# zepfu/llama-gguf-inference

Hardware: AMD Instinct MI355X
Metric: decode tokens/sec + achieved HBM GB/s, Llama-3-8B Q4_K_M, 1->8 MI355X (higher is better)
Workload: dtype int8; 1 GPU; llama3-8b-q4km: 128-token prompt -> greedy decode on the 128->640 trajectory, 1521 timed tokens at positions 133..1653 (mean context of the trajectory), 1 replica per GPU; model=llama3-8b-q4km, parallelism=replicas x1 (RCCL weight fan-out), global_batch=1

## Files before the change

llama-gguf-inference_amd/csrc/attn.hip:

```cpp
#include "kernels.h"
#include "attn_device.h"
#include "launch_util.h"

#include <cstdlib>

namespace llmi {

template <int D, int G>
__global__ __launch_bounds__(256) void k_attn_scores(AttnArgs a) {
    const int g = blockIdx.x, chunk = blockIdx.y;
    const int n_kv = a.st->pos + 1;
    const int t0 = chunk * 64;
    if (t0 >= n_kv) return;
    const int nt = min(64, n_kv - t0);
    __shared__ float qs[G][D];
    __shared__ __attribute__((aligned(16))) uint16_t ks[64][D + 8];
    for (int i = threadIdx.x; i < G * D; i += 256) qs[i / D][i % D] = h2f(f2h(a.q[(size_t)g * G * D + i]));
    constexpr int PPR = D * 2 / 16;
    const uint16_t* kb = a.kc + ((size_t)g * a.n_ctx + t0) * D;
    for (int i = threadIdx.x; i < nt * PPR; i += 256) {
        const int r = i / PPR, pc = i % PPR;
        *(u32x4*)&ks[r][pc * 8] = *(const u32x4*)(kb + (size_t)r * D + pc * 8);
    }
    __syncthreads();
// ... 585 lines not shown
                const double v = tb + j < n_kv ? (double)f : 0.0;
                if (j & 1) acc1 = __builtin_fma(v, (double)pr[j], acc1);
                else acc0 = __builtin_fma(v, (double)pr[j], acc0);
            }
        }
    }
    double acc = acc0 + acc1;
    acc += xor_partner_d<1>(acc);
    acc += xor_partner_d<2>(acc);
    if constexpr (SLV == 8) acc += xor_partner_d<4>(acc);
    if (sl == 0) a.out[(size_t)h * D + d] = (float)acc;
    LLMI_ATT_STAMP(0, 3)
}

template <int D, int G, int NP>
__global__ __launch_bounds__(256) void k_attl_scores(AttnArgs a) { attl_scores_body<D, G, NP>(a); }
__global__ __launch_bounds__(256) void k_attl_exp(AttnArgs a, int n_head, int kvb) { attl_exp_body(a, n_head, kvb); }
template <int D, int G>
__global__ __launch_bounds__(512) void k_attl_pv(AttnArgs a, int n_head, int kvb) { attl_pv_body<D, G>(a, n_head, kvb); }
template <int D>
__global__ __launch_bounds__(D) void k_attl_sum(AttnArgs a, int n_head) { attl_sum_body<D>(a, n_head); }

template <int D, int P, int S>
__global__ __launch_bounds__(512) void k_attn_d(AttnArgs a, int G, int HK, int kvb, int pf) {
    attn_d_body<D, P, S>(a, G, HK, kvb, pf & 1, (pf >> 1) & 1);
}

int g_xspin_limit = kXSpinLimit;
int g_xtag_skew = 0;

static int g_attn_s = 0;
static int g_attn_pf = 3;
int attn_d_slices(int n_head, int head_dim) {
    const int s = g_attn_s ? g_attn_s : n_head >= 128 ? 2 : n_head >= 64 ? 4 : 8;
    return head_dim / s >= 8 ? s : head_dim / 8;
}

static int g_attn_mode = 0;
void set_attn_mode(int mode) {
    g_attn_mode = mode;
    const char* e = getenv("LLMI_ATTN_S");
    const int v = e ? atoi(e) : 0;
    g_attn_s = (v == 2 || v == 4 || v == 8) ? v : 0;
    const char* f = getenv("LLMI_ATTN_PF");
    g_attn_pf = f ? atoi(f) : 1;
    const char* r = getenv("LLMI_ATTN_ROT");
    if (!r || atoi(r)) g_attn_pf |= 2;
}
// ... 82 lines not shown
    bool ok;
    switch (path) {
        case 1:
            ok = pick([&](auto D) { launch_k(k_attn_fused<D>, heads, dim3(1024), (size_t)kv_bound * 4, s, true, true, a, g, hk); }, d);
            break;
        case 2:
            ok = pick([&](auto D, auto G) {
                launch_k(k_attn_scores8<D, G>, dim3(hk, (kv_bound + 31) / 32), dim3(256), 0, s, true, false, a);
                launch_k(k_attn_pv16<D, G>, dim3(hk, D / 16), dim3(512), lds_g, s, false, true, a, kv_bound);
            }, d, gq);
            break;
        case 4:
            ok = pick([&](auto D, auto G, auto NP) {
                if constexpr (D == 64 || NP < 4)
                    launch_k(k_attn_x<D, G, NP>, dim3(hk, D / 16), dim3(512), lds_g, s, true, true, a, kv_bound);
            }, d, gq, Of<1, 2, 4>{attn_x_np(head_dim, kv_bound)});
            break;
        case 5:
            ok = pick([&](auto D, auto P) { launch_k(k_attn_r<D, P>, heads, dim3(512), 0, s, true, true, a, g, kv_bound); },
                      d, Of<1, 2, 4, 8>{attn_passes(kv_bound, 8)});
            break;
        case 6:
            ok = pick([&](auto D, auto P, auto S) {
                launch_k(k_attn_d<D, P, S>, dim3(n_head * S), dim3(512), 0, s, true, true, a, g, hk, kv_bound, g_attn_pf);
            }, d, Of<1, 2, 4, 8, 12, 16>{attn_passes(kv_bound, 16)}, Of<2, 4, 8>{attn_d_slices(n_head, head_dim)});
            break;
        case 7:
            ok = pick([&](auto D, auto G, auto NP) {
                launch_k(k_attl_scores<D, G, NP>, dim3(hk, lg.nscores), dim3(256), 0, s, true, false, a);
                launch_k(k_attl_exp, dim3(n_head, lg.ntile), dim3(256), 0, s, false, false, a, n_head, kv_bound);
                launch_k(k_attl_pv<D, G>, dim3(hk, lg.ntile), dim3(512), 0, s, false, false, a, n_head, kv_bound);
                launch_k(k_attl_sum<D>, heads, dim3(D), 0, s, false, true, a, n_head);
            }, d, gq, Of<1, 4>{lg.np});
            break;
        default:
            ok = pick([&](auto D, auto G) {
                launch_k(k_attn_scores<D, G>, dim3(hk, (kv_bound + 63) / 64), dim3(256), 0, s, true, false, a);
                launch_k(k_attn_pv<D, G>, dim3(hk, D / 16), dim3(256), 0, s, false, true, a);
            }, d, gq);
    }
    return ok ? hipGetLastError() : hipErrorInvalidValue;
}

}
```

llama-gguf-inference_amd/csrc/attn_device.h:

```cpp
#pragma once

#include "mv_device.h"

namespace llmi {

#if defined(LLMI_EXP_TRACE)
#define LLMI_ATT_STAMP(K, I)                                                                      \
    if (a.trace && (threadIdx.x & 63) == 0)                                                       \
        a.trace[((size_t)(K) * 4096 + blockIdx.y * gridDim.x + blockIdx.x) * 64 + (threadIdx.x >> 6) * 4 + (I)] = \
            __builtin_amdgcn_s_memrealtime();
#else
#define LLMI_ATT_STAMP(K, I)
#endif

template <int D, int G>
__device__ __forceinline__ void attn_scores8_body(const AttnArgs& a) {
    LLMI_ATT_STAMP(0, 0)
    const int g = blockIdx.x, tile = blockIdx.y, t0 = tile * 32;
    const int tid = threadIdx.x, lane = tid & 63, wave = tid >> 6;
    constexpr int DQ = D / 8;
    const int t = t0 + (tid >> 3), qd = tid & 7;
    const uint16_t* kr = a.kc + ((size_t)g * a.n_ctx + t) * D + qd * DQ;
    u32x4 kv[DQ / 8];
#pragma unroll
// ... 344 lines not shown
        if constexpr (SL == 8) v += xor_partner_d<4>(v);
        if (sl == 0) part[((size_t)(g * G + hh) * ntl + tile) * D + d] = v;
    }
}

template <int D>
__device__ __forceinline__ void attl_sum_body(const AttnArgs& a, int n_head) {
    const int h = blockIdx.x, d = threadIdx.x;
    const int n_kv = a.st->pos + 1;
    const int ntl = (a.n_ctx + kLongTile - 1) / kLongTile, ntv = (n_kv + kLongTile - 1) / kLongTile;
    const double* part = attl_part(a, n_head) + (size_t)h * ntl * D + d;
    double s = 0.0;
    for (int j0 = 0; j0 < ntv; j0 += 16) {
        double v[16];
#pragma unroll
        for (int k = 0; k < 16; ++k) v[k] = part[(size_t)min(j0 + k, ntl - 1) * D];
#pragma unroll
        for (int k = 0; k < 16; ++k)
            if (j0 + k < ntv) s += v[k];
    }
    a.out[(size_t)h * D + d] = (float)s;
}

template <int D, int P, int S>
__device__ __forceinline__ void attn_d_body(const AttnArgs& a, int G, int HK, int kvb, int pf = 0, int rot_on = 0) {
    constexpr int DQ = D / 8;
    constexpr int DS = D / S;
    constexpr int SLV = 512 / DS;
    constexpr int NVL = (64 * P + 8 * SLV - 1) / (8 * SLV);
    static_assert(SLV <= 64 && (SLV & (SLV - 1)) == 0, "PV lanes of a dim stay in one wave");
    __shared__ __attribute__((aligned(16))) float sp[64 * P + 8];
    __shared__ float redm[8];
    __shared__ double reds[8];
    LLMI_ATT_STAMP(0, 0)
    const int b = blockIdx.x, H = HK * G;
    const int g = b % HK, h = g * G + (b / HK) % G, ds = b / H;
    const int tid = threadIdx.x, lane = tid & 63, wave = tid >> 6;
    const int qd = tid & 7, pp = tid >> 3;
    const int pos = a.st->pos;
    const int lim = pf ? pos + 1 : kvb;
    const int rot = rot_on ? (b / HK) % P : 0;
    auto pb = [&](int p) { return p + rot < P ? p + rot : p + rot - P; };
    float4 qv[DQ / 4];
#pragma unroll
    for (int i = 0; i < DQ / 4; ++i) qv[i] = *(const float4*)(a.q + (size_t)h * D + qd * DQ + 4 * i);
    u32x4 kv[P][DQ / 8];
#pragma unroll
    for (int p = 0; p < P; ++p) {
        const int t = min(64 * pb(p) + pp, kvb - 1);
        const uint16_t* kr = a.kc + ((size_t)g * a.n_ctx + t) * D + qd * DQ;
        if (64 * pb(p) < lim) {
#pragma unroll
            for (int i = 0; i < DQ / 8; ++i) kv[p][i] = *(const u32x4*)(kr + 8 * i);
        } else {
#pragma unroll
            for (int i = 0; i < DQ / 8; ++i) kv[p][i] = u32x4{0u, 0u, 0u, 0u};
        }
    }
    const int d = ds * DS + tid / SLV, sl = tid % SLV;
    const uint16_t* vr = a.vc + ((size_t)g * D + d) * a.n_ctx;
    u32x4 vv[NVL];
#pragma unroll
    for (int u = 0; u < NVL; ++u) {
        if (8 * SLV * u < lim) vv[u] = *(const u32x4*)(vr + min(8 * sl + 8 * SLV * u, kvb - 8));
        else vv[u] = u32x4{0u, 0u, 0u, 0u};
    }
    const int n_kv = pos + 1;
    double q[DQ];
#pragma unroll
    for (int i = 0; i < DQ / 4; ++i) {
        q[4 * i + 0] = (double)h2f(f2h(qv[i].x)); q[4 * i + 1] = (double)h2f(f2h(qv[i].y));
        q[4 * i + 2] = (double)h2f(f2h(qv[i].z)); q[4 * i + 3] = (double)h2f(f2h(qv[i].w));
    }
    float m = -INFINITY;
#pragma unroll
    for (int p = 0; p < P; ++p) {
        if (64 * pb(p) >= lim) continue;
        double acc = 0.0;
#pragma unroll
        for (int i = 0; i < DQ / 8; ++i)
#pragma unroll
            for (int jj = 0; jj < 4; ++jj) {
                acc = __builtin_fma((double)h2f((uint16_t)kv[p][i][jj]), q[8 * i + 2 * jj], acc);
                acc = __builtin_fma((double)h2f((uint16_t)(kv[p][i][jj] >> 16)), q[8 * i + 2 * jj + 1], acc);
            }
        acc += xor_partner_d<1>(acc);
        acc += xor_partner_d<2>(acc);
        acc += xor_partner_d<4>(acc);
        const int t = 64 * pb(p) + pp;
// ... 66 lines not shown
```

llama-gguf-inference_amd/csrc/battn.hip:

```cpp
#include "kernels.h"
#include "attn_device.h"
#include "launch_util.h"

namespace llmi {

template <int D, int G>
__global__ __launch_bounds__(256) void k_battn_scores8(BAttnArgs b) {
    const AttnArgs a = b.a[blockIdx.z];
    attn_scores8_body<D, G>(a);
}
template <int D, int G>
__global__ __launch_bounds__(512) void k_battn_pv16(BAttnArgs b, int kvb) {
    const AttnArgs a = b.a[blockIdx.z];
    attn_pv16_body<D, G>(a, kvb);
}
template <int D, int P, int S>
__global__ __launch_bounds__(512) void k_battn_d(BAttnArgs b, int G, int HK, int kvb) {
    attn_d_body<D, P, S>(b.a[blockIdx.y], G, HK, kvb, 1, 1);
}
template <int D, int G, int NP>
__global__ __launch_bounds__(256) void k_battl_scores(BAttnArgs b) { attl_scores_body<D, G, NP>(b.a[blockIdx.z]); }
__global__ __launch_bounds__(256) void k_battl_exp(BAttnArgs b, int n_head, int kvb) { attl_exp_body(b.a[blockIdx.z], n_head, kvb); }
template <int D, int G>
__global__ __launch_bounds__(512) void k_battl_pv(BAttnArgs b, int n_head, int kvb) { attl_pv_body<D, G>(b.a[blockIdx.z], n_head, kvb); }
template <int D>
__global__ __launch_bounds__(D) void k_battl_sum(BAttnArgs b, int n_head) { attl_sum_body<D>(b.a[blockIdx.z], n_head); }

hipError_t launch_battention(const BAttnArgs& b, int nt, int n_head, int n_head_kv, int head_dim, int kv_bound,
                             hipStream_t s) {
    if (nt < 1 || nt > kMaxBatch || n_head_kv <= 0 || n_head % n_head_kv) return hipErrorInvalidValue;
    if (b.a[0].fa) return launch_battention_fa(b, nt, n_head, n_head_kv, head_dim, kv_bound, s);
    if (b.a[0].num) return launch_battention_x86(b, nt, n_head, n_head_kv, head_dim, kv_bound, s);
    const int g = n_head / n_head_kv, hk = n_head_kv;
    const OfD d{head_dim};
    const OfG gq{g};
    const LongGeo lg = attn_long_geo(kv_bound);
    bool ok = false;
    switch (battn_path(g, n_head, head_dim, kv_bound, nt)) {
        case 2:
            ok = pick([&](auto D, auto G) {
                hipLaunchKernelGGL((k_battn_scores8<D, G>), dim3(hk, (kv_bound + 31) / 32, nt), dim3(256), 0, s, b);
// ... 23 lines not shown
```

llama-gguf-inference_amd/csrc/mv_device.h:

```cpp
#pragma once

#include <hip/hip_runtime.h>

#include "kernels.h"
#include "../../include/llmi_math.h"

namespace llmi {

typedef unsigned int u32x4 __attribute__((ext_vector_type(4)));
typedef unsigned int u32x2 __attribute__((ext_vector_type(2)));
typedef int i32x4 __attribute__((ext_vector_type(4)));
typedef short short2_t __attribute__((ext_vector_type(2)));

#ifndef LLMI_NT
#define LLMI_NT 1
#endif
constexpr bool kNontemporalWeights = LLMI_NT != 0;

__device__ __forceinline__ float h2f(uint32_t h) {
    return (float)__builtin_bit_cast(_Float16, (uint16_t)(h & 0xffffu));
}
__device__ __forceinline__ uint16_t f2h(float f) {
    __asm__("" : "+v"(f));
    return __builtin_bit_cast(uint16_t, (_Float16)f);
// ... 178 lines not shown
        for (int j = 0; j < 16; ++j) am = fmaxf(am, fabsf(v[j]));
        am = fmaxf(am, xor_partner<1>(am));
        const float d = am / 127;
        if constexpr (X86) {
            const float id = am != 0.f ? 127.f / am : 0.0f;
#pragma unroll
            for (int j = 0; j < 16; ++j) q[j] = (int)__builtin_rintf(v[j] * id);
        } else {
            const float id = d != 0.f ? 1.0f / d : 0.0f;
#pragma unroll
            for (int j = 0; j < 16; ++j) q[j] = (int)roundf(v[j] * id);
        }
        uint8_t* rec = L.act + (size_t)(sb >> 4) * kRec;
        if ((sb & 1) == 0) *(float*)(rec + kRecBs + 2 * (sb & 15)) = h2f(f2h(d));
        u32x4 pk;
#pragma unroll
        for (int w = 0; w < 4; ++w)
            pk[w] = (uint32_t)(q[4 * w] & 0xff) | ((uint32_t)(q[4 * w + 1] & 0xff) << 8) |
                    ((uint32_t)(q[4 * w + 2] & 0xff) << 16) | ((uint32_t)(q[4 * w + 3] & 0xff) << 24);
        *(u32x4*)(rec + 16 * (sb & 15)) = pk;
    }
}

template <bool NORM, int NP>
struct ProRegs {
    float x[NP][16];
    float w[NORM ? NP : 1][16];
};
template <bool NORM, int NP, int NT = kMVThreads>
__device__ __forceinline__ void mv_prologue_issue(const MVArgs& A, ProRegs<NORM, NP>& R) {
    const int nsub = A.cols / 16;
#pragma unroll
    for (int i = 0; i < NP; ++i) {
        const int sb = min((int)threadIdx.x + i * NT, nsub - 1);
#pragma unroll
        for (int k = 0; k < 4; ++k) {
            const float4 xv = *(const float4*)(A.x + sb * 16 + 4 * k);
            R.x[i][4 * k + 0] = xv.x; R.x[i][4 * k + 1] = xv.y; R.x[i][4 * k + 2] = xv.z; R.x[i][4 * k + 3] = xv.w;
            if constexpr (NORM) {
                const float4 wv = *(const float4*)(A.nw + sb * 16 + 4 * k);
                R.w[i][4 * k + 0] = wv.x; R.w[i][4 * k + 1] = wv.y; R.w[i][4 * k + 2] = wv.z; R.w[i][4 * k + 3] = wv.w;
            }
        }
    }
}
template <bool NORM, int NP>
__device__ __forceinline__ void load_sub(const MVArgs& A, const ProRegs<NORM, NP>& R, int i, int sb, float (&v)[16],
                                         float (&w)[16]) {
    if (i < NP) {
#pragma unroll
        for (int ii = 0; ii < NP; ++ii)
            if (ii == i) {
#pragma unroll
// ... 51 lines not shown
            float v[16];
#pragma unroll
            for (int j = 0; j < 16; ++j) {
                v[j] = R.x[i][j];
                if constexpr (NORM) v[j] = (v[j] * scale) * R.w[i][j];
            }
            quant_sub<ACT, X86>(L, cols, sb, v);
        }
    }
    for (int sb = tid + NP * NT; sb < nsub; sb += NT) {
        float v[16], w[16];
        load_sub<NORM, NP>(A, R, NP, sb, v, w);
        if constexpr (NORM) {
#pragma unroll
            for (int j = 0; j < 16; ++j) v[j] = (v[j] * scale) * w[j];
        }
        quant_sub<ACT, X86>(L, cols, sb, v);
    }
}
template <int NI>
struct ImgRegs {
    u32x4 v[NI];
};
template <int NI, int NT = kMVThreads>
__device__ __forceinline__ void mv_img_issue(const MVArgs& A, ImgRegs<NI>& R) {
    const int n16 = (A.cols >> 8) * (kRec / 16);
#pragma unroll
    for (int i = 0; i < NI; ++i) R.v[i] = *(const u32x4*)(A.xq + 16 * min((int)threadIdx.x + i * NT, n16 - 1));
}
template <int NI, int NT = kMVThreads>
__device__ __forceinline__ void mv_img_finish(const MVArgs& A, const Lds& L, const ImgRegs<NI>& R) {
    const int n16 = (A.cols >> 8) * (kRec / 16);
#pragma unroll
    for (int i = 0; i < NI; ++i)
        if ((int)threadIdx.x + i * NT < n16) ((u32x4*)L.act)[threadIdx.x + i * NT] = R.v[i];
    for (int i = (int)threadIdx.x + NI * NT; i < n16; i += NT) ((u32x4*)L.act)[i] = *(const u32x4*)(A.xq + 16 * i);
}

template <int ACT, bool NORM, int X86 = 0>
__device__ __forceinline__ void mv_prologue(const MVArgs& A, const Lds& L) {
    ProRegs<NORM, 1> R;
    mv_prologue_issue<NORM, 1>(A, R);
    mv_prologue_finish<ACT, NORM, 1, kMVThreads, X86>(A, L, R);
}

constexpr uint32_t M4 = 0x0F0F0F0Fu, M2 = 0x03030303u, M1 = 0x01010101u;

__device__ __forceinline__ void scale_min(int j, uint32_t s0, uint32_t s1, uint32_t s2, int& sc, int& m) {
// ... 460 lines not shown

__device__ __forceinline__ float x86_v_expf(float x) {
    const float r = 0x1.8p23f;
    const float z = __builtin_fmaf(x, 0x1.715476p+0f, r);
    const float n = z - r;
    const float b = __builtin_fmaf(-n, 0x1.7f7d1cp-20f, __builtin_fmaf(-n, 0x1.62e4p-1f, x));
    const uint32_t e = __float_as_uint(z) << 23;
    const float k = __uint_as_float(e + __float_as_uint(1.0f));
    const float u = b * b;
    const float j = __builtin_fmaf(__builtin_fmaf(__builtin_fmaf(0x1.0e4020p-7f, b, 0x1.573e2ep-5f), u,
                                                  __builtin_fmaf(0x1.555e66p-3f, b, 0x1.fffdb6p-2f)),
                                   u, 0x1.ffffecp-1f * b);
    if (!(fabsf(n) > 126.f)) return __builtin_fmaf(j, k, k);
    const uint32_t g = n <= 0.f ? 0x82000000u : 0u;
    const float s1 = __uint_as_float(g + 0x7f000000u), s2 = __uint_as_float(e - g);
    if (fabsf(n) > 192.f) return s1 * s1;
    return __builtin_fmaf(s2, j, s2) * s1;
}
__device__ __forceinline__ float x86_silu(float x) { return x / (1.0f + x86_v_expf(-x)); }

struct TaskGeo {
    int lr, R, nj, U;
};
__host__ __device__ inline TaskGeo task_geo(const MVArgs& A) {
    TaskGeo g;
    g.lr = A.lr;
    g.R = A.rpt;
    g.U = A.cols >> 8;
    g.nj = (g.U + g.lr - 1) / g.lr;
    return g;
}

__host__ __device__ constexpr int q80_rs(int lr) { return 8 * lr + 4; }

template <int ACT>
__device__ __forceinline__ void fold_sub(float* F, int R, int lr, int n, bool last, float& acc) {
    constexpr int NC = row_chains<ACT>();
    const int lane = threadIdx.x & 63, nf = R * NC;
    const int len = ACT ? 8 * n : n, stride = ACT ? q80_rs(lr) : kq_cs(lr);
    for (int f = lane; f < nf; f += 64) {
        float a = chain_batched(len, acc, ChainAdd{F + f * stride});
        if (last) {
            F[kFoldF + f] = a;
            a = 0.f;
        }
        acc = a;
    }
// ... 245 lines not shown
        if constexpr (X86) {
            if constexpr (ACT == 1) {
                unit_store_x86<T_Q8_0>(load_unit<T_Q8_0>(sg, lu.row, lu.u, g.U), rec, F, r, ul, g.lr, g.R, lu.valid);
            } else {
                switch (sg.type) {
                    case T_Q4_K: unit_store_x86<T_Q4_K>(load_unit<T_Q4_K>(sg, lu.row, lu.u, g.U), rec, F, r, ul, g.lr, g.R, lu.valid); break;
                    case T_Q5_K: unit_store_x86<T_Q5_K>(load_unit<T_Q5_K>(sg, lu.row, lu.u, g.U), rec, F, r, ul, g.lr, g.R, lu.valid); break;
                    default: unit_store_x86<T_Q6_K>(load_unit<T_Q6_K>(sg, lu.row, lu.u, g.U), rec, F, r, ul, g.lr, g.R, lu.valid); break;
                }
            }
        } else if constexpr (ACT == 1) {
            unit_terms<T_Q8_0>(load_unit<T_Q8_0>(sg, lu.row, lu.u, g.U), rec, tm);
        } else {
            switch (sg.type) {
                case T_Q4_K: unit_terms<T_Q4_K>(load_unit<T_Q4_K>(sg, lu.row, lu.u, g.U), rec, tm); break;
                case T_Q5_K: unit_terms<T_Q5_K>(load_unit<T_Q5_K>(sg, lu.row, lu.u, g.U), rec, tm); break;
                default: unit_terms<T_Q6_K>(load_unit<T_Q6_K>(sg, lu.row, lu.u, g.U), rec, tm); break;
            }
        }
        sub_finish<ACT, EPI, MA, X86>(A, F, g, s, b, sg, tm, lu, r, ul, acc, vg, pos, best);
    }
}

__host__ __device__ inline TaskGeo task_geo_split(const MVArgs& A, int lanes, int R) {
    TaskGeo g;
    g.lr = lanes >> 1;
    g.R = R;
    g.U = A.cols >> 8;
    g.nj = (g.U + g.lr - 1) / g.lr;
    return g;
}
template <int T>
struct HalfW {
    u32x4 q[4];
    u32x4 s;
    u32x4 h[2];
    uint32_t d;
};
template <int T>
__device__ __forceinline__ HalfW<T> load_half(const Seg& sg, uint32_t row, uint32_t u, uint32_t U, uint32_t half) {
    static_assert(T == T_Q4_K || T == T_Q6_K, "split units: Q4_K and Q6_K");
    HalfW<T> w;
    const uint32_t P = (U * 16) << sg.rgs, ru = row * U + u;
    const uint32_t oa = piece_off(row, 0, u, U, 8, sg.rgs) + 4 * half * P;
#pragma unroll
    for (int p = 0; p < 4; ++p) w.q[p] = ldw(sg.a + oa + (uint32_t)p * P);
    if constexpr (T == T_Q4_K) {
// ... 216 lines not shown
```

llama-gguf-inference_amd/csrc/mv_kernels.h:

```cpp
#pragma once
#include "kernels.h"
#include "launch_util.h"
#include "mv_device.h"

#include <algorithm>
#include <cstdlib>
#include <map>
#include <mutex>
#include <tuple>
#include <type_traits>

namespace llmi {

#ifndef LLMI_MV_PINGPONG
#define LLMI_MV_PINGPONG 1
#endif
#ifndef LLMI_Q6_MASKED
#define LLMI_Q6_MASKED 1
#endif
constexpr bool kQ6Masked = LLMI_Q6_MASKED != 0;
__host__ inline size_t mv_lds_total(int act, int cols, int nw, int t, int t2, int x86 = 0) {
    const int ff = fold_stride_cols(act, x86, cols);
    const size_t base = fold_off(act, cols, nw) + (size_t)nw * ff * 4;
    return base + ((kQ6Masked && !x86 && (t == T_Q6_K || t2 == T_Q6_K)) ? (size_t)(cols >> 8) * kQ6MaskRec : 0);
}

static int g_split_by_pairs = getenv("LLMI_SPLIT_BY_PAIRS") ? atoi(getenv("LLMI_SPLIT_BY_PAIRS")) : 0;


#if defined(LLMI_EXP_TRACE)
#define MV_STAMP(I, V)                                                                                    \
    if (A.trace && (threadIdx.x & 63) == 0)                                                               \
        A.trace[((size_t)blockIdx.x * (NT / 64) + (threadIdx.x >> 6)) * 16 + (I)] = (V);
#define MV_NOW __builtin_amdgcn_s_memrealtime()
#else
#define MV_STAMP(I, V)
#endif

template <int ACT, bool NORM, int EPI, int T, int NP, int NT = kMVThreads, int X86 = 0, int US = 1>
__device__ __forceinline__ unsigned long long mv_body(const MVArgs& A, const Lds& L, float* F, const TaskGeo& g, int t0,
                                                      int G, int tbeg, int tend) {
    using W = std::conditional_t<US == 2, HalfW<US == 2 ? T : T_Q4_K>, UnitW<T>>;
    int pos = 0;
    if constexpr (EPI == EPI_QKV) pos = A.st->pos;
    unsigned long long best = 0;
    const int lane = threadIdx.x & 63;
    const int S = EPI == EPI_SWIGLU ? 2 * g.nj : g.nj;
    const int slot = US == 2 ? lane >> 1 : lane;
    [[maybe_unused]] const uint32_t half = lane & 1;
    const int r = slot / g.lr, ul = slot - r * g.lr;
    const auto load = [&](const Seg& s, uint32_t row, uint32_t u) {
        if constexpr (US == 2) return load_half<T>(s, row, u, g.U, half);
        else return load_unit<T>(s, row, u, g.U);
    };

    int task = t0;
    MV_STAMP(0, MV_NOW)
    [[maybe_unused]] int nsub_done = 0, nsub_alt = 0;
    ProRegs<NORM, NP> R;
    ImgRegs<2 * NP + 1> RI;
    const bool img = A.xq != nullptr;
    if (img) mv_img_issue<2 * NP + 1, NT>(A, RI);
    else mv_prologue_issue<NORM, NP, NT>(A, R);
    if ((tend - tbeg <= G && A.xfirst >= 0) || A.xfirst > 0) asm volatile("s_waitcnt vmcnt(0)" ::: "memory");
    const bool pipe = task < tend && task_is<EPI, T>(A, g, task);
    Sub b = sub_of<EPI>(A, g, task < tend ? task : tend - 1, 0);
    Seg sg = pick(A, b.si);
    LaneUnit lu = lane_unit(g, b, sg, r, ul);
    W cur = load(sg, pipe ? lu.row : 0u, pipe ? lu.u : 0u);
    if (img) mv_img_finish<2 * NP + 1, NT>(A, L, RI);
    else mv_prologue_finish<ACT, NORM, NP, NT, X86>(A, L, R);
    __syncthreads();
    [[maybe_unused]] uint8_t* q6m = nullptr;
    if constexpr (T == T_Q6_K && kQ6Masked && !X86) {
        q6m = (uint8_t*)L.act + fold_off(ACT, A.cols, NT / 64) + (size_t)(NT / 64) * kFoldFloats * 4;
        q6_masks_build<NT>(L, g.U, q6m);
        __syncthreads();
    }
    MV_STAMP(1, MV_NOW)

    if (pipe) {
        int s = 0;
        float acc = 0.f, vg = 0.f;
        bool first_sub = A.fw != 0;
        auto step = [&](W& cur, W& nxt) -> bool {
            int tn = task, sn = s + 1;
            Sub bn = b;
            Seg sgn = sg;
            bool has_next = true;
            if (sn == S) {
                sn = 0;
                tn = task + G;
                has_next = tn < tend && task_is<EPI, T>(A, g, tn);
            }
            if (has_next) {
                bn = sub_of<EPI>(A, g, tn, sn);
                sgn = pick(A, bn.si);
            }
// ... 39 lines not shown
            return true;
        };
#if LLMI_MV_PINGPONG
        W other;
        for (;;) {
            if (!step(cur, other)) break;
            if (!step(other, cur)) break;
        }
#else
        for (;;) {
            W nxt;
            if (!step(cur, nxt)) break;
            cur = nxt;
        }
#endif
    }
    if constexpr (US == 1)
        for (; task < tend; task += G) task_any<ACT, EPI, MVArgs, X86>(A, L, F, g, task, r, ul, pos, best);
    MV_STAMP(3, MV_NOW)
    MV_STAMP(5, ((unsigned long long)(__builtin_amdgcn_s_getreg(6164) & 15) << 32) | (unsigned)nsub_done)
    return best;
}

template <int ACT, bool NORM, int EPI, int T, int NP, int T2 = T, int NT = kMVThreads, int X86 = 0>
__global__ __launch_bounds__(NT) void k_matvec(MVArgs A) {
    constexpr int NW = NT / 64;
    extern __shared__ __attribute__((aligned(16))) uint8_t smem[];
    const Lds L = carve(smem, ACT, A.cols);
    const int wave = uniform((int)(threadIdx.x >> 6));
    const int lane = threadIdx.x & 63;
    float* F = (float*)(smem + fold_off(ACT, A.cols, NW)) + wave * fold_stride(ACT, X86, A.rpt, A.lr);
    unsigned long long best;
    if constexpr (T2 == T) {
        int t0 = blockIdx.x * NW + wave, G = gridDim.x * NW, tb = 0, te = A.ntasks;
        if (A.split_wgs > 0) {
            if ((int)blockIdx.x < A.split_wgs) {
                G = A.split_wgs * NW;
                te = A.split_tasks;
            } else {
                t0 = A.split_tasks + (blockIdx.x - A.split_wgs) * NW + wave;
                G = (gridDim.x - A.split_wgs) * NW;
                tb = A.split_tasks;
            }
        }
        best = mv_body<ACT, NORM, EPI, T, NP, NT, X86>(A, L, F, task_geo(A), t0, G, tb, te);
    } else {
        if ((int)blockIdx.x < A.split_wgs)
            best = mv_body<ACT, NORM, EPI, T, NP, NT, X86>(A, L, F, task_geo(A), blockIdx.x * NW + wave, A.split_wgs * NW, 0, A.split_tasks);
        else
            best = mv_body<ACT, NORM, EPI, T2, NP, NT, X86>(A, L, F, task_geo(A), A.split_tasks + (blockIdx.x - A.split_wgs) * NW + wave,
                                                            (gridDim.x - A.split_wgs) * NW, A.split_tasks, A.ntasks);
    }
    if constexpr (EPI == EPI_LOGITS) {
        const int cur_pos = A.st->pos;
        unsigned long long* red = (unsigned long long*)L.red;
        best = wave_max_u64(best);
        __syncthreads();
        if (lane == 0) red[wave] = best;
        __syncthreads();
        if (threadIdx.x == 0) {
            unsigned long long b = red[0];
#pragma unroll
            for (int w = 1; w < NW; ++w) b = red[w] > b ? red[w] : b;
            if (b) atomicMax(&A.argmax[(cur_pos & 1) * kArgSlots + blockIdx.x % kArgSlots], b);
            if (blockIdx.x == 0) A.st->pos_next = cur_pos + 1;
        }
    }
}

template <typename K>
static dim3 resident_grid(K kernel, dim3 grid, size_t lds, int threads = kMVThreads) {
    static std::mutex mu;
    static std::map<std::tuple<const void*, size_t, int>, int> cache;
    int dev = 0;
    (void)hipGetDevice(&dev);
    const auto key = std::make_tuple((const void*)kernel, lds, dev * 4096 + threads);
    int cap = 0;
    {
        std::lock_guard<std::mutex> lk(mu);
        auto it = cache.find(key);
        if (it != cache.end()) {
            cap = it->second;
        } else {
            int occ = 0, cus = 0;
            if (hipOccupancyMaxActiveBlocksPerMultiprocessor(&occ, kernel, threads, lds) != hipSuccess || occ <= 0) occ = 1;
            if (hipDeviceGetAttribute(&cus, hipDeviceAttributeMultiprocessorCount, dev) != hipSuccess || cus <= 0) cus = 1;
            cap = occ * cus;
            cache.emplace(key, cap);
        }
    }
// ... 9 lines not shown
    return v;
}
static inline int wide_cols() {
    static const int v = [] {
        const char* e = getenv("LLMI_MV_WIDE");
        return e ? atoi(e) : 12288;
    }();
    return v;
}
static inline int wide_epis() {
    static const int v = [] {
        const char* e = getenv("LLMI_MV_WIDE_EPI");
        return e ? atoi(e) : (1 << EPI_ADD) | (1 << EPI_SWIGLU) | (1 << EPI_QKV);
    }();
    return v;
}
constexpr int kMVWide = 512;
template <int ACT, bool NORM, int T, int EPI, int NP, int X86>
static hipError_t mv_launch_wide(const MVArgs& a, hipStream_t s) {
    constexpr int NW = kMVWide / 64;
    const size_t lds = mv_lds_total(ACT, a.cols, NW, T, T, X86);
    if (lds > 160 * 1024) return hipErrorInvalidValue;
    const int blocks = std::max(1, std::min(cu_count(), (a.ntasks + NW - 1) / NW));
    launch_k(k_matvec<ACT, NORM, EPI, T, NP, T, kMVWide, X86>, dim3(blocks), dim3(kMVWide), lds, s, true, true, a);
    return hipGetLastError();
}
template <int ACT, bool NORM, int T, int EPI, int X86>
static bool mv_try_wide(const MVArgs& a, hipStream_t s, hipError_t& e) {
    if constexpr ((EPI == EPI_ADD || EPI == EPI_SWIGLU || EPI == EPI_QKV || EPI == EPI_LOGITS) && !(X86 && ACT)) {
        const int wc = wide_cols();
        if (wc <= 0 || a.cols < wc || cu_count() <= 0 || !(wide_epis() >> EPI & 1)) return false;
        for (int i = 0; i < a.nseg; ++i)
            if (a.seg[i].type != T) return false;
        const int per = (a.cols / 16 + kMVWide - 1) / kMVWide;
        e = per <= 1 ? mv_launch_wide<ACT, NORM, T, EPI, 1, X86>(a, s)
            : per <= 2 ? mv_launch_wide<ACT, NORM, T, EPI, 2, X86>(a, s) : mv_launch_wide<ACT, NORM, T, EPI, 4, X86>(a, s);
        return true;
    } else {
        (void)a; (void)s; (void)e;
        return false;
    }
}
constexpr int kMVNarrow = 64;
static inline int narrow_on() {
    static const int v = getenv("LLMI_MV_NARROW") ? atoi(getenv("LLMI_MV_NARROW")) : 1;
    return v;
}
static inline int narrow_tpc() {
    static const int v = getenv("LLMI_MV_NARROW_TPC") ? atoi(getenv("LLMI_MV_NARROW_TPC")) : kMVWaves;
    return v;
}
template <int ACT, bool NORM, int T, int EPI, int NP, int X86>
static hipError_t mv_launch_narrow(const MVArgs& a0, hipStream_t s) {
    const size_t lds = mv_lds_total(ACT, a0.cols, 1, T, T, X86);
    if (lds > 160 * 1024) return hipErrorInvalidValue;
    auto k = k_matvec<ACT, NORM, EPI, T, NP, T, kMVNarrow, X86>;
    const dim3 g = resident_grid(k, dim3(a0.ntasks), lds, kMVNarrow);
    MVArgs a = a0;
    a.split_wgs = 0;
    launch_k(k, g, dim3(kMVNarrow), lds, s, true, true, a);
    return hipGetLastError();
}
template <int ACT, bool NORM, int T, int EPI, int X86>
static bool mv_try_narrow(const MVArgs& a, hipStream_t s, hipError_t& e) {
    if constexpr (EPI == EPI_ADD || EPI == EPI_SWIGLU || EPI == EPI_QKV || EPI == EPI_STORE) {
        const int cus = cu_count();
        if (!narrow_on() || cus <= 0 || a.ntasks >= cus * narrow_tpc()) return false;
        for (int i = 0; i < a.nseg; ++i)
            if (a.seg[i].type != T) return false;
        const int per = (a.cols / 16 + kMVNarrow - 1) / kMVNarrow;
        e = per <= 2 ? mv_launch_narrow<ACT, NORM, T, EPI, 2, X86>(a, s) : mv_launch_narrow<ACT, NORM, T, EPI, 4, X86>(a, s);
        return true;
    } else {
        (void)a; (void)s; (void)e;
        return false;
    }
}
template <int ACT, bool NORM, int T, int EPI, int NP, int X86>
static hipError_t mv_launch(const MVArgs& a0, dim3 grid, size_t lds_in, hipStream_t s) {
    const size_t lds = std::max(lds_in, mv_lds_total(ACT, a0.cols, kMVWaves, T, T, X86));
    if (lds > 160 * 1024) return hipErrorInvalidValue;
    auto k = k_matvec<ACT, NORM, EPI, T, NP, T, kMVThreads, X86>;
    const dim3 g = resident_grid(k, grid, lds);
    MVArgs a = a0;
    a.split_wgs = 0;
    const double sh = old_share();
    const int cus = cu_count();
    if (sh > 0 && cus > 0 && (int)g.x == 2 * cus && a.ntasks >= 4 * (int)g.x * kMVWaves) {
        a.split_wgs = cus;
        a.split_tasks = (int)(a.ntasks * (sh / (1.0 + sh)) + 0.5);
    }
    launch_k(k, g, dim3(kMVThreads), lds, s, true, true, a);
    return hipGetLastError();
}

static inline int split_groups(int wgs, int p1, int p2, double b1, double b2) {
    int best = 1;
    double best_cost = 1e300;
    for (int w1 = 1; w1 < wgs; ++w1) {
        const int n1 = w1 * kMVWaves, n2 = (wgs - w1) * kMVWaves;
        const double c = std::max((double)((p1 + n1 - 1) / n1) * b1, (double)((p2 + n2 - 1) / n2) * b2);
        if (c < best_cost) { best_cost = c; best = w1; }
    }
    return best;
}
template <int ACT, bool NORM, int T, int T2, int EPI, int NP, int X86>
static hipError_t mv_launch2(const MVArgs& a0, int split_tasks, dim3 grid, size_t lds_in, hipStream_t s) {
    const size_t lds = std::max(lds_in, mv_lds_total(ACT, a0.cols, kMVWaves, T, T2, X86));
    if (lds > 160 * 1024) return hipErrorInvalidValue;
    auto k = k_matvec<ACT, NORM, EPI, T, NP, T2, kMVThreads, X86>;
    const dim3 g = resident_grid(k, grid, lds);
    MVArgs a = a0;
    a.split_tasks = split_tasks;
    int w1;
    if (g_split_by_pairs) {
        w1 = (int)(((long long)g.x * split_tasks + a.ntasks / 2) / a.ntasks);
        w1 = w1 < 1 ? 1 : w1 > (int)g.x - 1 ? (int)g.x - 1 : w1;
    } else {
        w1 = split_groups((int)g.x, split_tasks, a.ntasks - split_tasks, (double)tensor_bytes(T, a.rpt, a.cols),
                          (double)tensor_bytes(T2, a.rpt, a.cols));
    }
    a.split_wgs = w1;
    launch_k(k, g, dim3(kMVThreads), lds, s, true, true, a);
    return hipGetLastError();
}

static inline int prologue_np(int cols) {
    const int per = (cols / 16 + kMVThreads - 1) / kMVThreads;
    return per <= 1 ? 1 : per <= 2 ? 2 : 4;
}

template <int ACT, bool NORM, int T, int EPI, int X86>
static hipError_t mv_launch_np(const MVArgs& a, dim3 grid, size_t lds, hipStream_t s) {
    hipError_t e = hipSuccess;
    if (mv_try_wide<ACT, NORM, T, EPI, X86>(a, s, e)) return e;
    if (mv_try_narrow<ACT, NORM, T, EPI, X86>(a, s, e)) return e;
    switch (prologue_np(a.cols)) {
        case 1: return mv_launch<ACT, NORM, T, EPI, 1, X86>(a, grid, lds, s);
        case 2: return mv_launch<ACT, NORM, T, EPI, 2, X86>(a, grid, lds, s);
        default: return mv_launch<ACT, NORM, T, EPI, 4, X86>(a, grid, lds, s);
    }
}

template <int ACT, bool NORM, int T, int X86>
hipError_t mv_dispatch_epi(const MVArgs& a, int epi, dim3 grid, size_t lds, hipStream_t s) {
    switch (epi) {
        case EPI_STORE: return mv_launch_np<ACT, NORM, T, EPI_STORE, X86>(a, grid, lds, s);
        case EPI_ADD: return mv_launch_np<ACT, NORM, T, EPI_ADD, X86>(a, grid, lds, s);
        default: break;
    }
    if constexpr (NORM) {
        switch (epi) {
            case EPI_QKV: return mv_launch_np<ACT, NORM, T, EPI_QKV, X86>(a, grid, lds, s);
            case EPI_SWIGLU: return mv_launch_np<ACT, NORM, T, EPI_SWIGLU, X86>(a, grid, lds, s);
            case EPI_LOGITS: return mv_launch_np<ACT, NORM, T, EPI_LOGITS, X86>(a, grid, lds, s);
            default: break;
        }
    }
    return hipErrorInvalidValue;
}

template <bool NORM, int T, int T2, int X86>
hipError_t mv_qkv2_launch(const MVArgs& a, int split_tasks, dim3 grid, size_t lds, hipStream_t s) {
    return mv_launch2<0, NORM, T, T2, EPI_QKV, 1, X86>(a, split_tasks, grid, lds, s);
}

template <bool NORM, int EPI, int T, int T2, int NT, int X86, int US, int US2>
__global__ __launch_bounds__(NT) void k_matvec_split(MVArgs A) {
    constexpr int NW = NT / 64;
    extern __shared__ __attribute__((aligned(16))) uint8_t smem[];
    const Lds L = carve(smem, 0, A.cols);
    const int wave = uniform((int)(threadIdx.x >> 6));
    float* F = (float*)(smem + fold_off(0, A.cols, NW)) + wave * fold_stride(0, X86, 1, 4);
    if constexpr (T2 == T) {
        static_assert(US == 2 && US2 == 2, "single-type split launches split every unit");
        mv_body<0, NORM, EPI, T, 1, NT, X86, 2>(A, L, F, task_geo_split(A, A.lr, A.rpt), blockIdx.x * NW + wave,
                                                 gridDim.x * NW, 0, A.ntasks);
    } else {
        if ((int)blockIdx.x < A.split_wgs) {
            const TaskGeo g = US == 2 ? task_geo_split(A, A.lr, A.rpt) : task_geo(A);
            mv_body<0, NORM, EPI, T, 1, NT, X86, US>(A, L, F, g, blockIdx.x * NW + wave, A.split_wgs * NW, 0, A.split_tasks);
        } else {
            const int bi = (int)blockIdx.x - A.split_wgs, nb2 = (int)gridDim.x - A.split_wgs;
            TaskGeo g = task_geo_split(A, A.lr2, A.rpt2);
            if constexpr (US2 == 1) {
                g.lr = A.lr2;
                g.nj = (g.U + g.lr - 1) / g.lr;
            }
            mv_body<0, NORM, EPI, T2, 1, NT, X86, US2>(A, L, F, g, A.t2beg + bi * NW + wave, nb2 * NW, A.t2beg, A.t2end);
        }
    }
}

template <bool NORM, int EPI, int T, int NT, int X86>
static hipError_t mv_split_launch_nt(const MVArgs& a, hipStream_t s) {
    constexpr int NW = NT / 64;
    const size_t lds = mv_lds_total(0, a.cols, NW, T, T, X86);
    if (lds > 160 * 1024) return hipErrorInvalidValue;
    auto k = k_matvec_split<NORM, EPI, T, T, NT, X86, 2, 2>;
    const dim3 g = resident_grid(k, dim3((a.ntasks + NW - 1) / NW), lds, NT);
    launch_k(k, g, dim3(NT), lds, s, true, true, a);
    return hipGetLastError();
}
template <bool NORM, int T, int X86>
hipError_t mv_split_launch(const MVArgs& a, int epi, int nt, hipStream_t s) {
    if (a.us != 2 || (nt != 256 && nt != 512)) return hipErrorInvalidValue;
    for (int i = 0; i < a.nseg; ++i)
        if (a.seg[i].type != T) return hipErrorInvalidValue;
#define LLMI_SPLIT_NT(E_) (nt == 512 ? mv_split_launch_nt<NORM, E_, T, 512, X86>(a, s) : mv_split_launch_nt<NORM, E_, T, 256, X86>(a, s))
    if (epi == EPI_STORE) return LLMI_SPLIT_NT(EPI_STORE);
    if (epi == EPI_ADD) return LLMI_SPLIT_NT(EPI_ADD);
    if constexpr (NORM)
        if (epi == EPI_QKV) return LLMI_SPLIT_NT(EPI_QKV);
#undef LLMI_SPLIT_NT
    return hipErrorInvalidValue;
}

static inline int split_groups_nw(int wgs, int nw, int p1, int p2, double b1, double b2) {
    int best = 1;
    double best_cost = 1e300;
    for (int w1 = 1; w1 < wgs; ++w1) {
        const int n1 = w1 * nw, n2 = (wgs - w1) * nw;
        const double c = std::max((double)((p1 + n1 - 1) / n1) * b1, (double)((p2 + n2 - 1) / n2) * b2);
        if (c < best_cost) { best_cost = c; best = w1; }
    }
    return best;
}
template <int NT, int X86, int US>
static hipError_t mv_split_qkv2_launch_nt(const MVArgs& a0, hipStream_t s) {
    constexpr int NW = NT / 64;
    const size_t lds = mv_lds_total(0, a0.cols, NW, T_Q4_K, T_Q6_K, X86);
    if (lds > 160 * 1024) return hipErrorInvalidValue;
    auto k = k_matvec_split<true, EPI_QKV, T_Q4_K, T_Q6_K, NT, X86, US, 2>;
    MVArgs a = a0;
    const int p1 = a.split_tasks, p2 = a.t2end - a.t2beg;
    const dim3 g = resident_grid(k, dim3((p1 + NW - 1) / NW + (p2 + NW - 1) / NW), lds, NT);
    if (g.x < 2) return hipErrorInvalidValue;
    a.split_wgs = split_groups_nw((int)g.x, NW, p1, p2, US == 2 ? 1.0 : 2.0, 2.4);
    launch_k(k, g, dim3(NT), lds, s, true, true, a);
    return hipGetLastError();
}
template <int X86, int US>
hipError_t mv_split_qkv2_launch(const MVArgs& a, int nt, hipStream_t s) {
    if (a.us != US || a.us2 != 2 || a.nseg < 2 || a.cols > 16 * 256 || (nt != 256 && nt != 512)) return hipErrorInvalidValue;
    return nt == 512 ? mv_split_qkv2_launch_nt<512, X86, US>(a, s) : mv_split_qkv2_launch_nt<256, X86, US>(a, s);
}

}
```

Measured before the change: 536.0 tokens/s.

## Hoist kernel-argument loads and overlap step-position read with early K-cache loads

Kernel arguments for the attention and matvec kernels are flattened into leading scalar parameters, so the hot fields sit at the front of the kernarg segment and can be loaded as scalars without pulling in the whole struct. In attention, the step position is now requested through an explicit scalar load, and for deep pass counts the K rows already known to be live are loaded before waiting on that position. The aim is to hide the latency of the dependent pos load and of the argument fetch at kernel start. The cost is more complex code with inline asm, a sched_barrier, and a 'live = kvb-256' margin that assumes pos never trails kvb by more than 256.

```diff
diff --git a/llama-gguf-inference_amd/csrc/attn.hip b/llama-gguf-inference_amd/csrc/attn.hip
--- a/llama-gguf-inference_amd/csrc/attn.hip
+++ b/llama-gguf-inference_amd/csrc/attn.hip
@@ -631,8 +631,12 @@
 __global__ __launch_bounds__(D) void k_attl_sum(AttnArgs a, int n_head) { attl_sum_body<D>(a, n_head); }
 
 template <int D, int P, int S>
-__global__ __launch_bounds__(512) void k_attn_d(AttnArgs a, int G, int HK, int kvb, int pf) {
-    attn_d_body<D, P, S>(a, G, HK, kvb, pf & 1, (pf >> 1) & 1);
+__global__ __launch_bounds__(512) void k_attn_d(const float* q, const uint16_t* kc, const uint16_t* vc, const StepState* st,
+                                                float* out, int n_ctx, int geo, int kvb, float scale,
+                                                unsigned long long* trace) {
+    const int pf = geo >> 24;
+    attn_d_body<D, P, S>(AttnDArgs{q, kc, vc, st, out, n_ctx, scale, trace}, geo & 255, (geo >> 8) & 0xffff, kvb, pf & 1,
+                         (pf >> 1) & 1);
 }
 
 int g_xspin_limit = kXSpinLimit;
@@ -761,7 +765,8 @@
             break;
         case 6:
             ok = pick([&](auto D, auto P, auto S) {
-                launch_k(k_attn_d<D, P, S>, dim3(n_head * S), dim3(512), 0, s, true, true, a, g, hk, kv_bound, g_attn_pf);
+                launch_k(k_attn_d<D, P, S>, dim3(n_head * S), dim3(512), 0, s, true, true, a.q, a.kc, a.vc, a.st, a.out,
+                         a.n_ctx, g | hk << 8 | g_attn_pf << 24, kv_bound, a.scale, a.trace);
             }, d, Of<1, 2, 4, 8, 12, 16>{attn_passes(kv_bound, 16)}, Of<2, 4, 8>{attn_d_slices(n_head, head_dim)});
             break;
         case 7:
diff --git a/llama-gguf-inference_amd/csrc/attn_device.h b/llama-gguf-inference_amd/csrc/attn_device.h
--- a/llama-gguf-inference_amd/csrc/attn_device.h
+++ b/llama-gguf-inference_amd/csrc/attn_device.h
@@ -390,8 +390,32 @@
     a.out[(size_t)h * D + d] = (float)s;
 }
 
+struct AttnDArgs {
+    const float* q;
+    const uint16_t* kc;
+    const uint16_t* vc;
+    const StepState* st;
+    float* out;
+    int n_ctx;
+    float scale;
+    unsigned long long* trace;
+};
+__device__ __forceinline__ AttnDArgs attn_d_args(const AttnArgs& a) {
+    return {a.q, a.kc, a.vc, a.st, a.out, a.n_ctx, a.scale, a.trace};
+}
+
+__device__ __forceinline__ int step_pos_request(const StepState* st) {
+    int pos;
+    asm volatile("s_load_dword %0, %1, %2" : "=s"(pos) : "s"(st), "n"(offsetof(StepState, pos)));
+    return pos;
+}
+__device__ __forceinline__ int step_pos_wait(int pos) {
+    asm volatile("s_waitcnt lgkmcnt(0)" : "+s"(pos));
+    return pos;
+}
+
 template <int D, int P, int S>
-__device__ __forceinline__ void attn_d_body(const AttnArgs& a, int G, int HK, int kvb, int pf = 0, int rot_on = 0) {
+__device__ __forceinline__ void attn_d_body(const AttnDArgs& a, int G, int HK, int kvb, int pf = 0, int rot_on = 0) {
     constexpr int DQ = D / 8;
     constexpr int DS = D / S;
     constexpr int SLV = 512 / DS;
@@ -400,29 +424,45 @@
     __shared__ __attribute__((aligned(16))) float sp[64 * P + 8];
     __shared__ float redm[8];
     __shared__ double reds[8];
+    const int pos_req = step_pos_request(a.st);
     LLMI_ATT_STAMP(0, 0)
     const int b = blockIdx.x, H = HK * G;
     const int g = b % HK, h = g * G + (b / HK) % G, ds = b / H;
     const int tid = threadIdx.x, lane = tid & 63, wave = tid >> 6;
     const int qd = tid & 7, pp = tid >> 3;
-    const int pos = a.st->pos;
-    const int lim = pf ? pos + 1 : kvb;
+    const int live = kvb - 256;
     const int rot = rot_on ? (b / HK) % P : 0;
     auto pb = [&](int p) { return p + rot < P ? p + rot : p + rot - P; };
     float4 qv[DQ / 4];
 #pragma unroll
     for (int i = 0; i < DQ / 4; ++i) qv[i] = *(const float4*)(a.q + (size_t)h * D + qd * DQ + 4 * i);
     u32x4 kv[P][DQ / 8];
+    auto k_row = [&](int p) {
+        const int t = min(64 * pb(p) + pp, kvb - 1);
+        return a.kc + ((size_t)g * a.n_ctx + t) * D + qd * DQ;
+    };
+    constexpr bool EARLY = P > 4;
+    if constexpr (EARLY) {
+#pragma unroll
+        for (int p = 0; p < P; ++p) {
+            if (64 * pb(p) + 64 <= live) {
+                const uint16_t* kr = k_row(p);
+#pragma unroll
+                for (int i = 0; i < DQ / 8; ++i) kv[p][i] = *(const u32x4*)(kr + 8 * i);
+            } else {
+#pragma unroll
+                for (int i = 0; i < DQ / 8; ++i) kv[p][i] = u32x4{0u, 0u, 0u, 0u};
+            }
+        }
+    }
+    const int pos = step_pos_wait(pos_req);
+    const int lim = pf ? pos + 1 : kvb;
 #pragma unroll
     for (int p = 0; p < P; ++p) {
-        const int t = min(64 * pb(p) + pp, kvb - 1);
-        const uint16_t* kr = a.kc + ((size_t)g * a.n_ctx + t) * D + qd * DQ;
-        if (64 * pb(p) < lim) {
+        if ((!EARLY || 64 * pb(p) + 64 > live) && 64 * pb(p) < lim) {
+            const uint16_t* kr = k_row(p);
 #pragma unroll
             for (int i = 0; i < DQ / 8; ++i) kv[p][i] = *(const u32x4*)(kr + 8 * i);
-        } else {
-#pragma unroll
-            for (int i = 0; i < DQ / 8; ++i) kv[p][i] = u32x4{0u, 0u, 0u, 0u};
         }
     }
     const int d = ds * DS + tid / SLV, sl = tid % SLV;
@@ -433,6 +473,7 @@
         if (8 * SLV * u < lim) vv[u] = *(const u32x4*)(vr + min(8 * sl + 8 * SLV * u, kvb - 8));
         else vv[u] = u32x4{0u, 0u, 0u, 0u};
     }
+    __builtin_amdgcn_sched_barrier(0);
     const int n_kv = pos + 1;
     double q[DQ];
 #pragma unroll
diff --git a/llama-gguf-inference_amd/csrc/battn.hip b/llama-gguf-inference_amd/csrc/battn.hip
--- a/llama-gguf-inference_amd/csrc/battn.hip
+++ b/llama-gguf-inference_amd/csrc/battn.hip
@@ -16,7 +16,7 @@
 }
 template <int D, int P, int S>
 __global__ __launch_bounds__(512) void k_battn_d(BAttnArgs b, int G, int HK, int kvb) {
-    attn_d_body<D, P, S>(b.a[blockIdx.y], G, HK, kvb, 1, 1);
+    attn_d_body<D, P, S>(attn_d_args(b.a[blockIdx.y]), G, HK, kvb, 1, 1);
 }
 template <int D, int G, int NP>
 __global__ __launch_bounds__(256) void k_battl_scores(BAttnArgs b) { attl_scores_body<D, G, NP>(b.a[blockIdx.z]); }
diff --git a/llama-gguf-inference_amd/csrc/mv_device.h b/llama-gguf-inference_amd/csrc/mv_device.h
--- a/llama-gguf-inference_amd/csrc/mv_device.h
+++ b/llama-gguf-inference_amd/csrc/mv_device.h
@@ -224,13 +224,22 @@
     }
 }
 
+struct MVLead {
+    const float* x;
+    const float* nw;
+    const uint8_t* xq;
+    StepState* st;
+    int cols, ntasks, split_wgs, split_tasks, lr, rpt;
+    int nwg;
+};
+
 template <bool NORM, int NP>
 struct ProRegs {
     float x[NP][16];
     float w[NORM ? NP : 1][16];
 };
-template <bool NORM, int NP, int NT = kMVThreads>
-__device__ __forceinline__ void mv_prologue_issue(const MVArgs& A, ProRegs<NORM, NP>& R) {
+template <bool NORM, int NP, int NT = kMVThreads, class MA>
+__device__ __forceinline__ void mv_prologue_issue(const MA& A, ProRegs<NORM, NP>& R) {
     const int nsub = A.cols / 16;
 #pragma unroll
     for (int i = 0; i < NP; ++i) {
@@ -328,8 +337,8 @@
 struct ImgRegs {
     u32x4 v[NI];
 };
-template <int NI, int NT = kMVThreads>
-__device__ __forceinline__ void mv_img_issue(const MVArgs& A, ImgRegs<NI>& R) {
+template <int NI, int NT = kMVThreads, class MA>
+__device__ __forceinline__ void mv_img_issue(const MA& A, ImgRegs<NI>& R) {
     const int n16 = (A.cols >> 8) * (kRec / 16);
 #pragma unroll
     for (int i = 0; i < NI; ++i) R.v[i] = *(const u32x4*)(A.xq + 16 * min((int)threadIdx.x + i * NT, n16 - 1));
@@ -836,7 +845,8 @@
 struct TaskGeo {
     int lr, R, nj, U;
 };
-__host__ __device__ inline TaskGeo task_geo(const MVArgs& A) {
+template <class MA>
+__host__ __device__ inline TaskGeo task_geo(const MA& A) {
     TaskGeo g;
     g.lr = A.lr;
     g.R = A.rpt;
@@ -1128,7 +1138,8 @@
     }
 }
 
-__host__ __device__ inline TaskGeo task_geo_split(const MVArgs& A, int lanes, int R) {
+template <class MA>
+__host__ __device__ inline TaskGeo task_geo_split(const MA& A, int lanes, int R) {
     TaskGeo g;
     g.lr = lanes >> 1;
     g.R = R;
diff --git a/llama-gguf-inference_amd/csrc/mv_kernels.h b/llama-gguf-inference_amd/csrc/mv_kernels.h
--- a/llama-gguf-inference_amd/csrc/mv_kernels.h
+++ b/llama-gguf-inference_amd/csrc/mv_kernels.h
@@ -38,11 +38,11 @@
 #endif
 
 template <int ACT, bool NORM, int EPI, int T, int NP, int NT = kMVThreads, int X86 = 0, int US = 1>
-__device__ __forceinline__ unsigned long long mv_body(const MVArgs& A, const Lds& L, float* F, const TaskGeo& g, int t0,
-                                                      int G, int tbeg, int tend) {
+__device__ __forceinline__ unsigned long long mv_body(const MVArgs& A, const MVLead& E, const Lds& L, float* F,
+                                                      const TaskGeo& g, int t0, int G, int tbeg, int tend) {
     using W = std::conditional_t<US == 2, HalfW<US == 2 ? T : T_Q4_K>, UnitW<T>>;
     int pos = 0;
-    if constexpr (EPI == EPI_QKV) pos = A.st->pos;
+    if constexpr (EPI == EPI_QKV) pos = E.st->pos;
     unsigned long long best = 0;
     const int lane = threadIdx.x & 63;
     const int S = EPI == EPI_SWIGLU ? 2 * g.nj : g.nj;
@@ -59,9 +59,9 @@
     [[maybe_unused]] int nsub_done = 0, nsub_alt = 0;
     ProRegs<NORM, NP> R;
     ImgRegs<2 * NP + 1> RI;
-    const bool img = A.xq != nullptr;
-    if (img) mv_img_issue<2 * NP + 1, NT>(A, RI);
-    else mv_prologue_issue<NORM, NP, NT>(A, R);
+    const bool img = E.xq != nullptr;
+    if (img) mv_img_issue<2 * NP + 1, NT>(E, RI);
+    else mv_prologue_issue<NORM, NP, NT>(E, R);
     if ((tend - tbeg <= G && A.xfirst >= 0) || A.xfirst > 0) asm volatile("s_waitcnt vmcnt(0)" ::: "memory");
     const bool pipe = task < tend && task_is<EPI, T>(A, g, task);
     Sub b = sub_of<EPI>(A, g, task < tend ? task : tend - 1, 0);
@@ -73,7 +73,7 @@
     __syncthreads();
     [[maybe_unused]] uint8_t* q6m = nullptr;
     if constexpr (T == T_Q6_K && kQ6Masked && !X86) {
-        q6m = (uint8_t*)L.act + fold_off(ACT, A.cols, NT / 64) + (size_t)(NT / 64) * kFoldFloats * 4;
+        q6m = (uint8_t*)L.act + fold_off(ACT, E.cols, NT / 64) + (size_t)(NT / 64) * kFoldFloats * 4;
         q6_masks_build<NT>(L, g.U, q6m);
         __syncthreads();
     }
@@ -159,34 +159,40 @@
     return best;
 }
 
+#define LLMI_MV_LEAD_PARAMS                                                                                        \
+    const float *x_, const float *nw_, const uint8_t *xq_, StepState *st_, int cols_, int ntasks_, int split_wgs_, \
+        int split_tasks_, int lr_rpt_, int nwg_
+#define LLMI_MV_LEAD MVLead { x_, nw_, xq_, st_, cols_, ntasks_, split_wgs_, split_tasks_, lr_rpt_ & 0xffff, lr_rpt_ >> 16, nwg_ }
+
 template <int ACT, bool NORM, int EPI, int T, int NP, int T2 = T, int NT = kMVThreads, int X86 = 0>
-__global__ __launch_bounds__(NT) void k_matvec(MVArgs A) {
+__global__ __launch_bounds__(NT) void k_matvec(LLMI_MV_LEAD_PARAMS, MVArgs A) {
+    const MVLead E = LLMI_MV_LEAD;
     constexpr int NW = NT / 64;
     extern __shared__ __attribute__((aligned(16))) uint8_t smem[];
-    const Lds L = carve(smem, ACT, A.cols);
+    const Lds L = carve(smem, ACT, E.cols);
     const int wave = uniform((int)(threadIdx.x >> 6));
     const int lane = threadIdx.x & 63;
-    float* F = (float*)(smem + fold_off(ACT, A.cols, NW)) + wave * fold_stride(ACT, X86, A.rpt, A.lr);
+    float* F = (float*)(smem + fold_off(ACT, E.cols, NW)) + wave * fold_stride(ACT, X86, E.rpt, E.lr);
     unsigned long long best;
     if constexpr (T2 == T) {
-        int t0 = blockIdx.x * NW + wave, G = gridDim.x * NW, tb = 0, te = A.ntasks;
-        if (A.split_wgs > 0) {
-            if ((int)blockIdx.x < A.split_wgs) {
-                G = A.split_wgs * NW;
-                te = A.split_tasks;
+        int t0 = blockIdx.x * NW + wave, G = E.nwg * NW, tb = 0, te = E.ntasks;
+        if (E.split_wgs > 0) {
+            if ((int)blockIdx.x < E.split_wgs) {
+                G = E.split_wgs * NW;
+                te = E.split_tasks;
             } else {
-                t0 = A.split_tasks + (blockIdx.x - A.split_wgs) * NW + wave;
-                G = (gridDim.x - A.split_wgs) * NW;
-                tb = A.split_tasks;
-            }
-        }
-        best = mv_body<ACT, NORM, EPI, T, NP, NT, X86>(A, L, F, task_geo(A), t0, G, tb, te);
+                t0 = E.split_tasks + (blockIdx.x - E.split_wgs) * NW + wave;
+                G = (E.nwg - E.split_wgs) * NW;
+                tb = E.split_tasks;
+            }
+        }
+        best = mv_body<ACT, NORM, EPI, T, NP, NT, X86>(A, E, L, F, task_geo(E), t0, G, tb, te);
     } else {
-        if ((int)blockIdx.x < A.split_wgs)
-            best = mv_body<ACT, NORM, EPI, T, NP, NT, X86>(A, L, F, task_geo(A), blockIdx.x * NW + wave, A.split_wgs * NW, 0, A.split_tasks);
+        if ((int)blockIdx.x < E.split_wgs)
+            best = mv_body<ACT, NORM, EPI, T, NP, NT, X86>(A, E, L, F, task_geo(E), blockIdx.x * NW + wave, E.split_wgs * NW, 0, E.split_tasks);
         else
-            best = mv_body<ACT, NORM, EPI, T2, NP, NT, X86>(A, L, F, task_geo(A), A.split_tasks + (blockIdx.x - A.split_wgs) * NW + wave,
-                                                            (gridDim.x - A.split_wgs) * NW, A.split_tasks, A.ntasks);
+            best = mv_body<ACT, NORM, EPI, T2, NP, NT, X86>(A, E, L, F, task_geo(E), E.split_tasks + (blockIdx.x - E.split_wgs) * NW + wave,
+                                                            (E.nwg - E.split_wgs) * NW, E.split_tasks, E.ntasks);
     }
     if constexpr (EPI == EPI_LOGITS) {
         const int cur_pos = A.st->pos;
@@ -203,6 +209,12 @@
             if (blockIdx.x == 0) A.st->pos_next = cur_pos + 1;
         }
     }
+}
+
+template <typename K>
+static void mv_launch_k(K kernel, dim3 grid, dim3 block, size_t lds, hipStream_t s, const MVArgs& a) {
+    launch_k(kernel, grid, block, lds, s, true, true, a.x, a.nw, a.xq, a.st, a.cols, a.ntasks, a.split_wgs, a.split_tasks,
+             a.lr | a.rpt << 16, (int)grid.x, a);
 }
 
 template <typename K>
@@ -258,7 +270,7 @@
     const size_t lds = mv_lds_total(ACT, a.cols, NW, T, T, X86);
     if (lds > 160 * 1024) return hipErrorInvalidValue;
     const int blocks = std::max(1, std::min(cu_count(), (a.ntasks + NW - 1) / NW));
-    launch_k(k_matvec<ACT, NORM, EPI, T, NP, T, kMVWide, X86>, dim3(blocks), dim3(kMVWide), lds, s, true, true, a);
+    mv_launch_k(k_matvec<ACT, NORM, EPI, T, NP, T, kMVWide, X86>, dim3(blocks), dim3(kMVWide), lds, s, a);
     return hipGetLastError();
 }
 template <int ACT, bool NORM, int T, int EPI, int X86>
@@ -294,7 +306,7 @@
     const dim3 g = resident_grid(k, dim3(a0.ntasks), lds, kMVNarrow);
     MVArgs a = a0;
     a.split_wgs = 0;
-    launch_k(k, g, dim3(kMVNarrow), lds, s, true, true, a);
+    mv_launch_k(k, g, dim3(kMVNarrow), lds, s, a);
     return hipGetLastError();
 }
 template <int ACT, bool NORM, int T, int EPI, int X86>
@@ -326,7 +338,7 @@
         a.split_wgs = cus;
         a.split_tasks = (int)(a.ntasks * (sh / (1.0 + sh)) + 0.5);
     }
-    launch_k(k, g, dim3(kMVThreads), lds, s, true, true, a);
+    mv_launch_k(k, g, dim3(kMVThreads), lds, s, a);
     return hipGetLastError();
 }
 
@@ -357,7 +369,7 @@
                           (double)tensor_bytes(T2, a.rpt, a.cols));
     }
     a.split_wgs = w1;
-    launch_k(k, g, dim3(kMVThreads), lds, s, true, true, a);
+    mv_launch_k(k, g, dim3(kMVThreads), lds, s, a);
     return hipGetLastError();
 }
 
@@ -402,28 +414,29 @@
 }
 
 template <bool NORM, int EPI, int T, int T2, int NT, int X86, int US, int US2>
-__global__ __launch_bounds__(NT) void k_matvec_split(MVArgs A) {
+__global__ __launch_bounds__(NT) void k_matvec_split(LLMI_MV_LEAD_PARAMS, MVArgs A) {
+    const MVLead E = LLMI_MV_LEAD;
     constexpr int NW = NT / 64;
     extern __shared__ __attribute__((aligned(16))) uint8_t smem[];
-    const Lds L = carve(smem, 0, A.cols);
+    const Lds L = carve(smem, 0, E.cols);
     const int wave = uniform((int)(threadIdx.x >> 6));
-    float* F = (float*)(smem + fold_off(0, A.cols, NW)) + wave * fold_stride(0, X86, 1, 4);
+    float* F = (float*)(smem + fold_off(0, E.cols, NW)) + wave * fold_stride(0, X86, 1, 4);
     if constexpr (T2 == T) {
         static_assert(US == 2 && US2 == 2, "single-type split launches split every unit");
-        mv_body<0, NORM, EPI, T, 1, NT, X86, 2>(A, L, F, task_geo_split(A, A.lr, A.rpt), blockIdx.x * NW + wave,
-                                                 gridDim.x * NW, 0, A.ntasks);
+        mv_body<0, NORM, EPI, T, 1, NT, X86, 2>(A, E, L, F, task_geo_split(E, E.lr, E.rpt), blockIdx.x * NW + wave,
+                                                 E.nwg * NW, 0, E.ntasks);
     } else {
-        if ((int)blockIdx.x < A.split_wgs) {
-            const TaskGeo g = US == 2 ? task_geo_split(A, A.lr, A.rpt) : task_geo(A);
-            mv_body<0, NORM, EPI, T, 1, NT, X86, US>(A, L, F, g, blockIdx.x * NW + wave, A.split_wgs * NW, 0, A.split_tasks);
+        if ((int)blockIdx.x < E.split_wgs) {
+            const TaskGeo g = US == 2 ? task_geo_split(E, E.lr, E.rpt) : task_geo(E);
+            mv_body<0, NORM, EPI, T, 1, NT, X86, US>(A, E, L, F, g, blockIdx.x * NW + wave, E.split_wgs * NW, 0, E.split_tasks);
         } else {
-            const int bi = (int)blockIdx.x - A.split_wgs, nb2 = (int)gridDim.x - A.split_wgs;
-            TaskGeo g = task_geo_split(A, A.lr2, A.rpt2);
+            const int bi = (int)blockIdx.x - E.split_wgs, nb2 = E.nwg - E.split_wgs;
+            TaskGeo g = task_geo_split(E, A.lr2, A.rpt2);
             if constexpr (US2 == 1) {
                 g.lr = A.lr2;
                 g.nj = (g.U + g.lr - 1) / g.lr;
             }
-            mv_body<0, NORM, EPI, T2, 1, NT, X86, US2>(A, L, F, g, A.t2beg + bi * NW + wave, nb2 * NW, A.t2beg, A.t2end);
+            mv_body<0, NORM, EPI, T2, 1, NT, X86, US2>(A, E, L, F, g, A.t2beg + bi * NW + wave, nb2 * NW, A.t2beg, A.t2end);
         }
     }
 }
@@ -435,7 +448,7 @@
     if (lds > 160 * 1024) return hipErrorInvalidValue;
     auto k = k_matvec_split<NORM, EPI, T, T, NT, X86, 2, 2>;
     const dim3 g = resident_grid(k, dim3((a.ntasks + NW - 1) / NW), lds, NT);
-    launch_k(k, g, dim3(NT), lds, s, true, true, a);
+    mv_launch_k(k, g, dim3(NT), lds, s, a);
     return hipGetLastError();
 }
 template <bool NORM, int T, int X86>
@@ -473,7 +486,7 @@
     const dim3 g = resident_grid(k, dim3((p1 + NW - 1) / NW + (p2 + NW - 1) / NW), lds, NT);
     if (g.x < 2) return hipErrorInvalidValue;
     a.split_wgs = split_groups_nw((int)g.x, NW, p1, p2, US == 2 ? 1.0 : 2.0, 2.4);
-    launch_k(k, g, dim3(NT), lds, s, true, true, a);
+    mv_launch_k(k, g, dim3(NT), lds, s, a);
     return hipGetLastError();
 }
 template <int X86, int US>
```

Measured after the change: 546.1 tokens/s, median of 6. 1.02x the previous value.
